# TissueImageAnalytics/cerberus

Hardware: AMD Instinct MI355X
Metric: Mpx/sec WSI tiled inference (all heads) (higher is better)
Workload: dtype f32

## Files before the change

cerberus_amd/build.py:

```python
import os
import subprocess
import sys

HERE = os.path.dirname(os.path.abspath(__file__))
CSRC = os.path.join(HERE, "csrc")
LIB = os.path.join(HERE, "libcerberus_hip.so")
LIB_DEV = os.path.join(HERE, "libcerberus_hip_dev.so")
LIB_HOST = os.path.join(HERE, "libcerberus_host.so")
HOST_SOURCES = ["host_codecs.c"]
SOURCES = ["conv_igemm.hip", "conv_wino.hip", "conv_wino4.hip", "conv_wino4b.hip", "conv_wino4p.hip", "net_kernels.hip", "postproc.hip", "slide_kernels.hip", "train_kernels.hip", "head_train.hip", "conv_wgrad.hip", "conv_wgrad_wino.hip", "pack_kernels.hip", "targets.hip", "valid_stats.hip", "jpeg_kernels.hip", "tissue_mask.hip", "cerb_api.hip", "cerb_train.hip"]
DEV_SOURCES = ["cerb_api.hip", "cerb_train.hip", "postproc.hip", "conv_wino4b.hip", "train_kernels.hip", "net_kernels.hip"]
DEV_ONLY_SOURCES = ["dev_entry.hip"]
FLAGS = ["--offload-arch=gfx950", "-O3", "-std=c++17", "-fPIC", "-Wall", "-Wno-unused-function", "-Wno-unused-result"]
EXTRA_FLAGS = {"conv_wino4.hip": ["-mllvm", "-pragma-unroll-threshold=1000000", "-mllvm", "-amdgpu-mfma-vgpr-form"],
               "conv_wino4b.hip": ["-mllvm", "-pragma-unroll-threshold=1000000"],
               "conv_wino4p.hip": ["-mllvm", "-pragma-unroll-threshold=1000000"]}


def _stale(target, deps):
    if not os.path.exists(target):
        return True
    t = os.path.getmtime(target)
    return any(os.path.getmtime(d) > t for d in deps if os.path.exists(d))


def build_host(force=False, verbose=True):
    srcs = [os.path.join(CSRC, f) for f in HOST_SOURCES]
    if force or _stale(LIB_HOST, srcs + [os.path.join(os.path.dirname(HERE), "include", "cerberus_host.h")]):
        cmd = [os.environ.get("CC", "gcc"), "-O3", "-std=c11", "-fPIC", "-shared", "-Wall", "-Wextra", "-pthread", "-o", LIB_HOST] + srcs + ["-lz"]
        if verbose:
            print(" ".join(cmd), flush=True)
        subprocess.check_call(cmd)
    return LIB_HOST


def build(force=False, verbose=True):
    build_host(force, verbose)
    hipcc = os.environ.get("HIPCC", "/opt/rocm/bin/hipcc")
    headers = [os.path.join(CSRC, f) for f in os.listdir(CSRC) if f.endswith(".h")]
    headers.append(os.path.join(os.path.dirname(HERE), "include", "cerberus_hip.h"))
    objs = []
    procs = []
    for src in SOURCES:
        sp = os.path.join(CSRC, src)
        if not os.path.exists(sp):
            continue
        obj = os.path.join(CSRC, src.replace(".hip", ".o"))
        objs.append(obj)
        if force or _stale(obj, [sp] + headers):
            cmd = [hipcc] + FLAGS + EXTRA_FLAGS.get(src, []) + ["-c", sp, "-o", obj]
            if verbose:
                print(" ".join(cmd), flush=True)
            procs.append((src, subprocess.Popen(cmd)))
    dev_objs = list(objs)
    for src in DEV_SOURCES:
        sp = os.path.join(CSRC, src)
        if not os.path.exists(sp):
            continue
        obj = os.path.join(CSRC, "dev_" + src.replace(".hip", ".o"))
        dev_objs[dev_objs.index(os.path.join(CSRC, src.replace(".hip", ".o")))] = obj
        if force or _stale(obj, [sp] + headers):
            cmd = [hipcc] + FLAGS + ["-DCERB_DEV_SWITCHES"] + EXTRA_FLAGS.get(src, []) + ["-c", sp, "-o", obj]
            if verbose:
                print(" ".join(cmd), flush=True)
            procs.append((src + " (dev)", subprocess.Popen(cmd)))
    for src in DEV_ONLY_SOURCES:
        sp = os.path.join(CSRC, src)
        obj = os.path.join(CSRC, "dev_" + src.replace(".hip", ".o"))
        dev_objs.append(obj)
        if force or _stale(obj, [sp] + headers):
            cmd = [hipcc] + FLAGS + ["-DCERB_DEV_SWITCHES"] + EXTRA_FLAGS.get(src, []) + ["-c", sp, "-o", obj]
            if verbose:
                print(" ".join(cmd), flush=True)
            procs.append((src + " (dev)", subprocess.Popen(cmd)))
    for src, p in procs:
        if p.wait() != 0:
            raise RuntimeError("hipcc failed on %s" % src)
    for lib, lobjs in ((LIB, objs), (LIB_DEV, dev_objs)):
        if force or procs or _stale(lib, lobjs):
            cmd = [hipcc, "--offload-arch=gfx950", "-shared", "-fPIC", "-o", lib] + lobjs
            if verbose:
                print(" ".join(cmd), flush=True)
            subprocess.check_call(cmd)
    return LIB


if __name__ == "__main__":
    build(force="--force" in sys.argv)
    print(LIB)
```

cerberus_amd/csrc/cerb_api.hip:

```cpp
#include "cerb_net.h"

static thread_local std::string g_err;
int cerb_set_error(const std::string& m) {
    g_err = m;
    return 1;
}
extern "C" int cerb_version(void) { return 1; }
extern "C" const char* cerb_last_error(void) { return g_err.c_str(); }
std::atomic<long long> g_devbuf_bytes{0};
extern "C" size_t cerb_device_bytes_held(void) { const long long v = g_devbuf_bytes.load(); return v > 0 ? (size_t)v : 0; }
thread_local hipStream_t g_call_stream = nullptr;

static int alloc_dev(cerb_net* net, size_t bytes, void** out) {
    if (net->reusing) {
        if (net->reuse_cursor >= net->n_finalize_allocs || net->dev_alloc_bytes[net->reuse_cursor] != bytes)
            return fail("reload: the tensors do not have the shapes the handle was finalized with");
        *out = net->dev_allocs[net->reuse_cursor++];
        return 0;
    }
    void* d = nullptr;
    HIP_OK(hipMalloc(&d, bytes));
    net->dev_allocs.push_back(d);
    net->dev_alloc_bytes.push_back(bytes);
    *out = d;
// ... 541 lines not shown
        if (!out) return 0;
    }
    const double fl = 2.0 * (double)c.groups * N * p.Ho * p.Wo * (double)c.cout * c.cin * c.ks * c.ks;
    const long long map_px = (long long)p.Ho * p.Wo;
    const bool use_w4 = net->conv_algo == 5 || net->conv_algo == 7 || (net->conv_algo == 6 && map_px >= 256);
    const bool planar = planar_out_gs > 0;
    static const long long w4b_max_px = [] {
        const char* e = cerb_dev_getenv("CERB_W4B_MAX_PX");
        return e ? atoll(e) : 4096ll;
    }();
    const bool w4b = !planar && (net->conv_algo == 7 || (net->conv_algo == 6 && map_px <= w4b_max_px)) && c.cin % 64 == 0;
    if (planar && !(use_w4 && c.wino && mode == 0 && net->fold_bn && !resid)) return fail("internal: conv " + name + " cannot take the planar path");
    if (use_w4 && c.wino && mode == 0 && (!it->second.host_w.empty() || !net->fold_bn)) {
        PackedConv& cm = it->second;
        float* train_slot = nullptr;
        if (!net->fold_bn && train_wino4_slot(net, name, cm, w4b ? 1 : 0, 0, st, &train_slot)) return 1;
        float*& slot4 = !net->fold_bn ? train_slot : (w4b ? cm.wino4b : cm.wino4);
        if (!slot4) {
            std::vector<float> w4;
            for (int g = 0; g < cm.groups; ++g) pack_wino4(cm.host_w.data() + (size_t)g * cm.cout * cm.cin * 9, cm.cout, cm.cin, &w4, w4b ? 1 : 0);
            void* d = nullptr;
            HIP_OK(hipMalloc(&d, w4.size() * 4));
            net->dev_allocs.push_back(d);
            net->dev_alloc_bytes.push_back(w4.size() * 4);
            HIP_OK(hipMemcpy(d, w4.data(), w4.size() * 4, hipMemcpyHostToDevice));
            slot4 = (float*)d;
        }
        p.wpack = slot4;
        p.w_gs = (long long)c.cout * c.cin * 36;
        double fl_done = fl;
        if (roi && roi[1] > roi[0] && roi[3] > roi[2]) {
            p.roi_y0 = roi[0]; p.roi_y1 = roi[1]; p.roi_x0 = roi[2]; p.roi_x1 = roi[3];
            const double ty = (roi[1] + 15) / 16 - roi[0] / 16, tx = (roi[3] + 15) / 16 - roi[2] / 16;
            fl_done = fl * (ty * 16.0 * tx * 16.0) / ((double)p.Ho * p.Wo);
        }
        if (planar) {
            p.out_gs = planar_out_gs;
            p.level_tag = net->planar_half ? 0 : 1;
            p.pl_byp = cerb_planar_blocks(p.Ho);
            p.pl_bxp = cerb_planar_blocks(p.Wo);
        }
        if (prof_begin(net, name, planar ? (p.level_tag ? "conv_wino4p<f4x4,16x16x2,planar>" : "conv_wino4p<f4x4,16x16x2,planar,half-res>") : w4b ? (cerb_wino4b_packed(p) ? (resid ? "conv_wino4b<f4x4,16t,res>" : "conv_wino4b<f4x4,16t>") : (resid ? "conv_wino4b<f4x4,16x16,res>" : "conv_wino4b<f4x4,16x16>")) : (resid ? "conv_wino4<f4x4,16x16x2,res>" : "conv_wino4<f4x4,16x16x2>"), fl_done, st)) return 1;
        if (net->conv_bn_part && !planar && !resid && !(roi && roi[1] > roi[0] && roi[3] > roi[2])) {
            p.bn_part = net->conv_bn_part;
            net->conv_bn_bpg = w4b ? cerb_wino4b_bn_blocks(p) : N * ((p.Ho + 15) / 16) * ((p.Wo + 15) / 16);
        }
        HIP_OK(planar ? cerb_launch_wino4p(p, st) : w4b ? cerb_launch_wino4b(p, st) : cerb_launch_wino4(p, st));
        if (prof_end(net, st)) return 1;
        return 0;
    }
    if (net->conv_algo && c.wino && mode == 0) {
        if (train_wino2_fresh(net, name, it->second, 0, st)) return 1;
        p.wpack = c.wino;
        p.w_gs = (long long)c.cout * c.cin * 16;
        double fl_done = fl;
        if (roi && roi[1] > roi[0] && roi[3] > roi[2]) {
            p.roi_y0 = roi[0]; p.roi_y1 = roi[1]; p.roi_x0 = roi[2]; p.roi_x1 = roi[3];
            const double ty = (roi[1] + 7) / 8 - roi[0] / 8, tx = (roi[3] + 15) / 16 - roi[2] / 16;
            fl_done = fl * (ty * 8.0 * tx * 16.0) / ((double)p.Ho * p.Wo);
        }
        if (prof_begin(net, name, resid ? "conv_wino<f2x2,8x16,res>" : "conv_wino<f2x2,8x16>", fl_done, st)) return 1;
        HIP_OK(cerb_launch_wino(p, st));
        if (prof_end(net, st)) return 1;
        return 0;
    }
    const std::string kn = "conv_igemm<ks" + std::to_string(c.ks) + ",s" + std::to_string(c.stride) + ",mode" + std::to_string(mode) +
                           (p.Wo < 32 ? ",16x16>" : ",8x32>");
    if (prof_begin(net, name, kn, fl, st)) return 1;
    HIP_OK(cerb_launch_conv(p, c.ks, c.stride, mode, st));
    if (prof_end(net, st)) return 1;
    return 0;
}

static int forward_impl(cerb_net* net, const cerb_forward_io* io, hipStream_t st, double* macs) {
    g_call_stream = st;
    const bool dry = (macs != nullptr) && (io->tiles == nullptr) && (io->tiles_f32 == nullptr);
    const int N = io->n, H = io->h, W = io->w;
    if (N <= 0 || H <= 0 || W <= 0 || (H % 16) || (W % 16)) return fail("cerb_net_forward: tile H,W must be positive multiples of 16");
    const int out_h = io->out_h > 0 ? io->out_h : H, out_w = io->out_w > 0 ? io->out_w : W;
    if (out_h > H || out_w > W) return fail("cerb_net_forward: crop larger than tile");
    const int hs[5] = {H, H / 2, H / 4, H / 8, H / 16}, ws[5] = {W, W / 2, W / 4, W / 8, W / 16};
    const size_t D = net->trunk_idx.size();
    const size_t guard = cerb_conv_guard_bytes(W);
    auto level_is_planar = [&](int u) {
        if (dry || u < 2 || !net->planar || !net->fold_bn || net->conv_algo != 6 || net->head_algo < 1) return false;
        const std::string n0 = "dec." + std::to_string(u) + ".0", n1 = "dec." + std::to_string(u) + ".1";
        auto c0 = net->conv.find(n0), c1 = net->conv.find(n1);
        if (c0 == net->conv.end() || c1 == net->conv.end() || !c0->second.wino) return false;
        return (long long)hs[3 - u] * ws[3 - u] > 4096 && c0->second.cin == 64 && c0->second.cout == 64 && c1->second.cout == 64;
    };
    if (!dry) {
        if (net->x0.ensure((size_t)N * H * W * 64 * 4, guard) || net->pool.ensure((size_t)N * hs[1] * ws[1] * 64 * 4, guard)) return fail_alloc();
        for (int i = 1; i < 5; ++i)
            if (net->x[i].ensure((size_t)N * hs[i] * ws[i] * kFilters[i] * 4, guard)) return fail_alloc();
        if (net->ta.ensure((size_t)N * hs[1] * ws[1] * 64 * 4, guard) || net->tb.ensure((size_t)N * hs[1] * ws[1] * 64 * 4, guard) ||
            net->cm.ensure((size_t)N * hs[4] * ws[4] * 256 * 4, guard))
            return fail_alloc();
        if (D) {
            static const bool exact_ws = cerb_dev_getenv("CERB_LEGACY_WS") == nullptr;
            size_t need_sum = 0, need_mid = 0;
            const int oc[4] = {128, 64, 64, 64};
            for (int u = 0; u < 4; ++u) {
                if (exact_ws && level_is_planar(u)) continue;
                const std::string n0 = "dec." + std::to_string(u) + ".0";
                auto c0 = net->conv.find(n0);
                const size_t px = (size_t)D * N * hs[3 - u] * ws[3 - u];
                need_sum = std::max(need_sum, px * (size_t)(c0 != net->conv.end() ? c0->second.cin : 256) * 4);
                need_mid = std::max(need_mid, px * (size_t)(c0 != net->conv.end() ? c0->second.cout : 256) * 4);
            }
            if (!exact_ws) need_sum = need_mid = D * (size_t)N * H * W * 64 * 4;
            if (net->dmid.ensure(need_mid, guard)) return fail_alloc();
            if (net->conv_algo && net->dsum.ensure(need_sum, guard)) return fail_alloc();
            for (int u = 0; u < 4; ++u) {
                if (exact_ws && level_is_planar(u)) continue;
                if (net->dout[u].ensure(D * (size_t)N * hs[3 - u] * ws[3 - u] * oc[u] * 4, guard)) return fail_alloc();
            }
        }
    }
    if (macs) *macs += (double)N * H * W * 64.0 * 147.0;
    if (!dry) {
        StemParams sp;
        sp.tiles = io->tiles; sp.tiles_f32 = io->tiles ? nullptr : io->tiles_f32; sp.wpack = net->stem_w; sp.bias = net->stem_b; sp.out = net->x0.p; sp.N = N; sp.H = H; sp.W = W; sp.relu = 1;
        sp.tiles_x = sp.tiles_y = 0;
        if (prof_begin(net, "stem", "stem_conv7x7", 2.0 * N * H * W * 64.0 * 147.0, st)) return 1;
        HIP_OK(cerb_launch_stem(sp, st));
        if (prof_end(net, st)) return 1;
        if (prof_begin(net, "maxpool", "maxpool3x3s2", 0.0, st)) return 1;
        HIP_OK(cerb_launch_maxpool(net->x0.p, net->pool.p, N, H, W, 64, st));
        if (prof_end(net, st)) return 1;
    }
    float* cur = dry ? nullptr : net->pool.p;
    int inpl = 64;
    for (int li = 0; li < 4; ++li) {
        const int planes = kFilters[li + 1];
        const int Hi = (li == 0) ? hs[1] : hs[li], Wi = (li == 0) ? ws[1] : ws[li];
        for (int b = 0; b < kLayers[li]; ++b) {
            const std::string p = "backbone.layer" + std::to_string(li + 1) + "." + std::to_string(b);
            const int stride = (b == 0 && li > 0) ? 2 : 1;
            const int hin = (b == 0) ? Hi : hs[li + 1], win = (b == 0) ? Wi : ws[li + 1];
            float* t1 = dry ? nullptr : net->ta.p;
            const bool last = (b == kLayers[li] - 1);
            float* outb = dry ? nullptr : (((kLayers[li] - 1 - b) % 2 == 0) ? net->x[li + 1].p : net->tb.p);
            (void)last;
            const float* idt = cur;
            if (run_conv(net, p + ".conv1", cur, nullptr, nullptr, t1, N, hin, win, 1, 0, 0, 0, st, macs)) return 1;
            if (stride != 1 || inpl != planes) {
                float* ds = dry ? nullptr : net->pool.p;
                if (run_conv(net, p + ".downsample", cur, nullptr, nullptr, ds, N, hin, win, 0, 0, 0, 0, st, macs)) return 1;
                idt = ds;
            }
            if (run_conv(net, p + ".conv2", t1, nullptr, idt, outb, N, hs[li + 1], ws[li + 1], 1, 0, 0, 0, st, macs)) return 1;
            cur = outb;
            inpl = planes;
        }
    }
    if (run_conv(net, "conv_map", dry ? nullptr : net->x[4].p, nullptr, nullptr, dry ? nullptr : net->cm.p, N, hs[4], ws[4], 0, 0, 0, 0, st, macs)) return 1;

    const long long tile_stride = io->tile_stride ? io->tile_stride : (long long)out_h * out_w;
    const long long row_stride = io->row_stride ? io->row_stride : out_w;
    if (net->pc_idx >= 0) {
        if (macs) *macs += (double)N * (512.0 * 256 + 256.0 * net->dec[net->pc_idx].out_ch);
        const bool want = io->out && io->out[net->pc_idx];
        const bool wantl = io->logits && io->logits[net->pc_idx];
        if (!dry && (want || wantl)) {
            PatchClassParams pp;
            memset(&pp, 0, sizeof(pp));
            pp.x4 = net->x[4].p; pp.bn1_s = net->pc_bn1s; pp.bn1_b = net->pc_bn1b; pp.w1t = net->pc_w1t; pp.b1 = net->pc_b1;
            pp.w2t = net->pc_w2t; pp.b2 = net->pc_b2;
            pp.N = N; pp.Hf = hs[4]; pp.Wf = ws[4]; pp.out_ch = net->dec[net->pc_idx].out_ch;
            pp.out_h = out_h; pp.out_w = out_w;
            pp.logits = wantl ? io->logits[net->pc_idx] : nullptr;
            pp.out = want ? (float*)io->out[net->pc_idx] : nullptr;
            pp.tile_off = io->tile_off; pp.tile_stride = tile_stride; pp.row_stride = row_stride;
            if (prof_begin(net, "patch_class", "patch_class", 2.0 * N * (512.0 * 256 + 256.0 * pp.out_ch), st)) return 1;
            HIP_OK(cerb_launch_patch_class(pp, st));
            if (prof_end(net, st)) return 1;
        }
    }
    if (D) {
        const float* skips[4] = {dry ? nullptr : net->x[3].p, dry ? nullptr : net->x[2].p, dry ? nullptr : net->x[1].p, dry ? nullptr : net->x0.p};
        const float* prev = dry ? nullptr : net->cm.p;
        long long prev_gs = 0;
        const int oc[4] = {128, 64, 64, 64};
        int roi_out[4][4], roi_mid[4][4], roi_sum[4][4];
        const bool any_logits = [&] {
            if (!io->logits) return false;
            for (size_t k = 0; k < net->dec.size(); ++k)
                if (io->logits[k]) return true;
            return false;
        }();
        const bool use_roi = !dry && net->crop_roi && (net->conv_algo == 1 || net->conv_algo >= 5) && !any_logits && (out_h < H || out_w < W);
        if (use_roi) {
            int y0 = (int)((H - out_h) * 0.5), x0 = (int)((W - out_w) * 0.5), y1 = y0 + out_h, x1 = x0 + out_w;
            for (int u = 3; u >= 0; --u) {
                const int hh = hs[3 - u], ww = ws[3 - u];
                auto widen = [&](int* r, const int* in, int d) {
                    r[0] = std::max(0, (in[0] - d) & ~3); r[1] = std::min(hh, (in[1] + d + 3) & ~3);
                    r[2] = std::max(0, (in[2] - d) & ~3); r[3] = std::min(ww, (in[3] + d + 3) & ~3);
                };
                const int win[4] = {y0, y1, x0, x1};
                widen(roi_out[u], win, 0);
                widen(roi_mid[u], roi_out[u], 1);
                widen(roi_sum[u], roi_mid[u], 1);
                y0 = std::max(0, roi_sum[u][0] / 2 - 1); y1 = std::min(hh / 2, (roi_sum[u][1] - 1) / 2 + 2);
                x0 = std::max(0, roi_sum[u][2] / 2 - 1); x1 = std::min(ww / 2, (roi_sum[u][3] - 1) / 2 + 2);
            }
        }
        bool feat_planar = false, prev_planar = false;
        for (int u = 0; u < 4; ++u) {
            const int hh = hs[3 - u], ww = ws[3 - u];
            const std::string n0 = "dec." + std::to_string(u) + ".0", n1 = "dec." + std::to_string(u) + ".1";
            const int cmid = net->conv[n0].cout;
            const int cin0 = net->conv[n0].cin;
            const bool lvl_planar = level_is_planar(u) && (u == 3 || prev_gs > 0);
            if (lvl_planar) {
                PlanarBuf &bs = u == 3 ? net->psum : net->psum2, &bm = u == 3 ? net->pmid : net->pmid2, &bo = bs;
                if (bs.ensure((int)D, N, hh, ww, 64, st) || bm.ensure((int)D, N, hh, ww, 64, st)) return fail_alloc();
                if (prof_begin(net, n0 + ".up", "upsample2_add_planar", 0.0, st)) return 1;
                HIP_OK(cerb_launch_upsample2_add_planar(skips[u], prev, bs.b.p, (int)D, N, hh, ww, cin0, prev_gs, bs.gs(), use_roi ? roi_sum[u] : nullptr, prev_planar ? 1 : 0, st));
                if (prof_end(net, st)) return 1;
                net->planar_half = (u != 3);
                if (run_conv(net, n0, bs.b.p, nullptr, nullptr, bm.b.p, N, hh, ww, 1, 0, bs.gs(), 0, st, macs, use_roi ? roi_mid[u] : nullptr, bm.gs()))
                    return 1;
                if (run_conv(net, n1, bm.b.p, nullptr, nullptr, bo.b.p, N, hh, ww, 1, 0, bm.gs(), 0, st, macs, use_roi ? roi_out[u] : nullptr, bo.gs()))
                    return 1;
                if (u == 3) feat_planar = true;
                prev = bo.b.p;
                prev_gs = bo.gs();
                prev_planar = true;
                continue;
            }
            if (prev_planar) return fail("internal: a tile-planar decoder level feeds an NHWC one");
            if (net->conv_algo && net->conv[n0].wino && !dry) {
                if (prof_begin(net, n0 + ".up", "upsample2_add", 0.0, st)) return 1;
                HIP_OK(cerb_launch_upsample2_add(skips[u], prev, net->dsum.p, (int)D, N, hh, ww, cin0, prev_gs, use_roi ? roi_sum[u] : nullptr, st));
                if (prof_end(net, st)) return 1;
                if (run_conv(net, n0, net->dsum.p, nullptr, nullptr, net->dmid.p, N, hh, ww, 1, 0, (long long)N * hh * ww * cin0, 0, st, macs,
                             use_roi ? roi_mid[u] : nullptr))
                    return 1;
            } else if (run_conv(net, n0, skips[u], prev, nullptr, dry ? nullptr : net->dmid.p, N, hh, ww, 1, 1, 0, prev_gs, st, macs)) return 1;
            if (run_conv(net, n1, dry ? nullptr : net->dmid.p, nullptr, nullptr, dry ? nullptr : net->dout[u].p, N, hh, ww, 1, 0,
                         (long long)N * hh * ww * cmid, 0, st, macs, use_roi ? roi_out[u] : nullptr))
                return 1;
            prev = dry ? nullptr : net->dout[u].p;
            prev_gs = (long long)N * hh * ww * oc[u];
        }
        HeadParams hps[8];
        int n_hp = 0;
        double head_flops = 0.0;
        for (size_t k = 0; k < net->dense_idx.size(); ++k) {
            const int di = net->dense_idx[k];
            const size_t tk = (size_t)net->trunk_of[k];
            const DecoderCfg& d = net->dec[di];
            if (macs) *macs += (double)N * H * W * (64.0 * 96 + 96.0 * d.out_ch);
            const bool want = io->out && io->out[di];
            const bool wantl = io->logits && io->logits[di];
            if (dry || !(want || wantl)) continue;
            HeadParams hp;
            memset(&hp, 0, sizeof(hp));
            hp.feat = feat_planar ? net->psum.b.p + tk * net->psum.gs() : net->dout[3].p + tk * (size_t)N * H * W * 64;
            hp.feat_planar = feat_planar ? 1 : 0;
            hp.pl_byp = cerb_planar_blocks(H);
            hp.pl_bxp = cerb_planar_blocks(W);
            hp.w1p = net->head_w1[k]; hp.b1 = net->head_b1[k]; hp.w2p = net->head_w2[k]; hp.b2 = net->head_b2[k]; hp.w2q = net->head_w2q[k];
            hp.N = N; hp.H = H; hp.W = W; hp.out_ch = d.out_ch; hp.kind = d.kind;
            hp.crop_y0 = (int)((H - out_h) * 0.5); hp.crop_x0 = (int)((W - out_w) * 0.5);
            hp.out_h = want ? out_h : 0; hp.out_w = want ? out_w : 0;
            hp.roi = use_roi ? 1 : 0;
            hp.logits = wantl ? io->logits[di] : nullptr;
            hp.absmax_bits = io->logit_absmax ? io->logit_absmax + di : nullptr;
            if (want) {
                if (d.kind == 0) hp.out_inst = (float*)io->out[di];
                else if (io->type_is_u8) hp.out_type_u8 = (unsigned char*)io->out[di];
                else hp.out_type_i64 = (long long*)io->out[di];
            }
            hp.tile_off = io->tile_off; hp.tile_stride = tile_stride; hp.row_stride = row_stride;
            const double head_px = hp.roi ? (double)out_h * (((hp.crop_x0 + out_w + 15) / 16 - hp.crop_x0 / 16) * 16.0) : (double)H * W;
            const double fl = 2.0 * N * head_px * (64.0 * 96 + 96.0 * d.out_ch);
            if (net->head_algo == 0) {
                if (prof_begin(net, "head." + d.name, "head", fl, st)) return 1;
                HIP_OK(cerb_launch_head(hp, st));
                if (prof_end(net, st)) return 1;
            } else {
                if (n_hp == 8) {
                    if (prof_begin(net, "heads", "head_group", head_flops, st)) return 1;
                    HIP_OK(cerb_launch_head_group(hps, n_hp, st, net->head_algo == 1 ? 1 : 0));
                    if (prof_end(net, st)) return 1;
                    n_hp = 0;
                    head_flops = 0.0;
                }
                hps[n_hp++] = hp;
                head_flops += fl;
            }
        }
        if (n_hp > 0) {
            if (prof_begin(net, "heads", "head_group", head_flops, st)) return 1;
            HIP_OK(cerb_launch_head_group(hps, n_hp, st, net->head_algo == 1 ? 1 : 0));
            if (prof_end(net, st)) return 1;
        }
    }
    if (!dry && io->feats) {
        const float* src[6] = {net->x0.p, net->x[1].p, net->x[2].p, net->x[3].p, net->cm.p, net->x[4].p};
        const size_t nb[6] = {(size_t)N * H * W * 64, (size_t)N * hs[1] * ws[1] * 64, (size_t)N * hs[2] * ws[2] * 128,
                              (size_t)N * hs[3] * ws[3] * 256, (size_t)N * hs[4] * ws[4] * 256, (size_t)N * hs[4] * ws[4] * 512};
        for (int i = 0; i < 6; ++i)
            if (io->feats[i]) HIP_OK(hipMemcpyAsync(io->feats[i], src[i], nb[i] * 4, hipMemcpyDeviceToDevice, st));
    }
    return 0;
}

extern "C" int cerb_net_begin_reload(cerb_net* net) {
    if (!net) return fail("cerb_net_begin_reload: null handle");
    HIP_OK(hipDeviceSynchronize());
    while (net->dev_allocs.size() > net->n_finalize_allocs) {
        (void)hipFree(net->dev_allocs.back());
        net->dev_allocs.pop_back();
        net->dev_alloc_bytes.pop_back();
    }
    net->reusing = true;
    net->reuse_cursor = 0;
// ... 195 lines not shown
```

cerberus_amd/csrc/net_kernels.hip:

```cpp
#include "cerb_common.h"

struct StemParams {
    const unsigned char* tiles;
    const float* tiles_f32;
    const float* wpack;
    const float* bias;
    float* out;
    int N, H, W, tiles_x, tiles_y;
    int relu;
};

template <bool F32IN>
__global__ __launch_bounds__(256, 2) void stem_conv7x7_kernel(StemParams p) {
    constexpr int TH = 8, TW = 32, IH = TH + 6, IW = TW + 6, ROW = 120;
    __shared__ __attribute__((aligned(16))) float wl[7 * 12 * 2 * 64];
    __shared__ __attribute__((aligned(16))) float xl[IH * ROW];
    const int tid = threadIdx.x, lane = tid & 63, wave = tid >> 6, j = lane & 31, h = lane >> 5;
    for (int i = tid; i < 7 * 12 * 2 * 64; i += 256) wl[i] = p.wpack[i];
    const int ntile = p.N * p.tiles_y * p.tiles_x;
    for (int tile = blockIdx.x; tile < ntile; tile += gridDim.x) {
        int t_ = tile;
        const int tx = t_ % p.tiles_x;
        t_ /= p.tiles_x;
        const int ty = t_ % p.tiles_y;
        const int n = t_ / p.tiles_y;
        const int oy0 = ty * TH, ox0 = tx * TW;
        __syncthreads();
        const unsigned char* img = F32IN ? nullptr : p.tiles + (long long)n * p.H * p.W * 3;
        const float* imgf = F32IN ? p.tiles_f32 + (long long)n * p.H * p.W * 3 : nullptr;
        for (int i = tid; i < IH * ROW; i += 256) {
            const int iy = i / ROW, c = i % ROW;
            const int gy = oy0 - 3 + iy, gx = ox0 - 3 + c / 3;
            float v = 0.f;
            if (c < IW * 3 && gy >= 0 && gy < p.H && gx >= 0 && gx < p.W) {
                const long long at = ((long long)gy * p.W + gx) * 3 + c % 3;
                v = (F32IN ? imgf[at] : (float)img[at]) / 255.0f;
            }
            xl[i] = v;
        }
        __syncthreads();
        f32x16 acc[2][2];
#pragma unroll
        for (int s = 0; s < 2; ++s)
#pragma unroll
            for (int q = 0; q < 2; ++q)
#pragma unroll
                for (int r = 0; r < 16; ++r) acc[s][q][r] = 0.f;
        const int b0 = (wave * 2 + 0) * ROW + j * 3 + h;
        const int b1 = (wave * 2 + 1) * ROW + j * 3 + h;
#pragma unroll
        for (int ky = 0; ky < 7; ++ky) {
#pragma unroll
            for (int t = 0; t < 12; ++t) {
                const float a0 = wl[((ky * 12 + t) * 2 + 0) * 64 + lane];
                const float a1 = wl[((ky * 12 + t) * 2 + 1) * 64 + lane];
                const float x0 = xl[b0 + ky * ROW + 2 * t];
                const float x1 = xl[b1 + ky * ROW + 2 * t];
                acc[0][0] = __builtin_amdgcn_mfma_f32_32x32x2f32(a0, x0, acc[0][0], 0, 0, 0);
                acc[1][0] = __builtin_amdgcn_mfma_f32_32x32x2f32(a1, x0, acc[1][0], 0, 0, 0);
                acc[0][1] = __builtin_amdgcn_mfma_f32_32x32x2f32(a0, x1, acc[0][1], 0, 0, 0);
                acc[1][1] = __builtin_amdgcn_mfma_f32_32x32x2f32(a1, x1, acc[1][1], 0, 0, 0);
            }
        }
#pragma unroll
        for (int q = 0; q < 2; ++q) {
            const int oy = oy0 + wave * 2 + q, ox = ox0 + j;
            if (oy >= p.H || ox >= p.W) continue;
            float* o = p.out + (((long long)n * p.H + oy) * p.W + ox) * 64;
#pragma unroll
            for (int s = 0; s < 2; ++s)
#pragma unroll
                for (int rq = 0; rq < 4; ++rq) {
                    const int co = s * 32 + rq * 8 + h * 4;
                    f32x4 v = {acc[s][q][rq * 4 + 0], acc[s][q][rq * 4 + 1], acc[s][q][rq * 4 + 2], acc[s][q][rq * 4 + 3]};
                    v = v + *reinterpret_cast<const f32x4*>(p.bias + co);
                    const float floor_ = p.relu ? 0.f : -3.402823466e38f;
                    v[0] = fmaxf(v[0], floor_);
                    v[1] = fmaxf(v[1], floor_);
                    v[2] = fmaxf(v[2], floor_);
                    v[3] = fmaxf(v[3], floor_);
                    *reinterpret_cast<f32x4*>(o + co) = v;
                }
        }
    }
}

hipError_t cerb_launch_stem(StemParams p, hipStream_t st) {
    p.tiles_x = (p.W + 31) / 32;
    p.tiles_y = (p.H + 7) / 8;
    const long long ntile = (long long)p.N * p.tiles_x * p.tiles_y;
    const unsigned grid = (unsigned)(ntile < 256 * 6 ? ntile : 256 * 6);
    if (p.tiles) hipLaunchKernelGGL(stem_conv7x7_kernel<false>, dim3(grid), dim3(256), 0, st, p);
    else hipLaunchKernelGGL(stem_conv7x7_kernel<true>, dim3(grid), dim3(256), 0, st, p);
    return hipGetLastError();
}

__global__ void maxpool3x3s2_kernel(const float* __restrict__ in, float* __restrict__ out, int N, int H, int W, int C, int Ho, int Wo) {
    const long long total = (long long)N * Ho * Wo * (C / 4);
    const long long per_xcd = gridDim.x / 8, vb = (long long)(blockIdx.x & 7) * per_xcd + (blockIdx.x >> 3);
    for (long long i = vb * (long long)blockDim.x + threadIdx.x; i < total; i += (long long)gridDim.x * blockDim.x) {
        const int c4 = (int)(i % (C / 4));
        long long r = i / (C / 4);
        const int ox = (int)(r % Wo);
        r /= Wo;
        const int oy = (int)(r % Ho);
        const int n = (int)(r / Ho);
        f32x4 m = {-INFINITY, -INFINITY, -INFINITY, -INFINITY};
#pragma unroll
        for (int ky = 0; ky < 3; ++ky) {
            const int y = oy * 2 - 1 + ky;
            if (y < 0 || y >= H) continue;
#pragma unroll
            for (int kx = 0; kx < 3; ++kx) {
                const int x = ox * 2 - 1 + kx;
                if (x < 0 || x >= W) continue;
                const f32x4 v = *reinterpret_cast<const f32x4*>(in + (((long long)n * H + y) * W + x) * C + c4 * 4);
                m[0] = fmaxf(m[0], v[0]);
                m[1] = fmaxf(m[1], v[1]);
                m[2] = fmaxf(m[2], v[2]);
                m[3] = fmaxf(m[3], v[3]);
            }
        }
        *reinterpret_cast<f32x4*>(out + i * 4) = m;
    }
}

__global__ void maxpool3x3s2_idx_kernel(const float* __restrict__ in, float* __restrict__ out, unsigned* __restrict__ idx, int N, int H, int W, int C, int Ho, int Wo) {
    const long long total = (long long)N * Ho * Wo * (C / 4);
    const long long per_xcd = gridDim.x / 8, vb = (long long)(blockIdx.x & 7) * per_xcd + (blockIdx.x >> 3);
    for (long long i = vb * (long long)blockDim.x + threadIdx.x; i < total; i += (long long)gridDim.x * blockDim.x) {
        const int c4 = (int)(i % (C / 4));
        long long r = i / (C / 4);
        const int ox = (int)(r % Wo);
        r /= Wo;
        const int oy = (int)(r % Ho);
        const int n = (int)(r / Ho);
        f32x4 m = {-INFINITY, -INFINITY, -INFINITY, -INFINITY};
        unsigned w0 = 0, w1 = 0, w2 = 0, w3 = 0;
        bool first = true;
#pragma unroll
        for (int ky = 0; ky < 3; ++ky) {
            const int y = oy * 2 - 1 + ky;
            if (y < 0 || y >= H) continue;
#pragma unroll
            for (int kx = 0; kx < 3; ++kx) {
                const int x = ox * 2 - 1 + kx;
                if (x < 0 || x >= W) continue;
                const f32x4 v = *reinterpret_cast<const f32x4*>(in + (((long long)n * H + y) * W + x) * C + c4 * 4);
                const unsigned k = (unsigned)(ky * 3 + kx);
                if (first || v[0] > m[0]) w0 = k;
                if (first || v[1] > m[1]) w1 = k;
                if (first || v[2] > m[2]) w2 = k;
                if (first || v[3] > m[3]) w3 = k;
                first = false;
                m[0] = fmaxf(m[0], v[0]);
                m[1] = fmaxf(m[1], v[1]);
                m[2] = fmaxf(m[2], v[2]);
                m[3] = fmaxf(m[3], v[3]);
            }
        }
        *reinterpret_cast<f32x4*>(out + i * 4) = m;
        idx[i] = w0 | (w1 << 8) | (w2 << 16) | (w3 << 24);
    }
}

hipError_t cerb_launch_maxpool_idx(const float* in, float* out, unsigned* idx, int N, int H, int W, int C, hipStream_t st) {
    const int Ho = (H + 2 - 3) / 2 + 1, Wo = (W + 2 - 3) / 2 + 1;
    const long long total = (long long)N * Ho * Wo * (C / 4);
    long long blocks = ((total + 255) / 256 + 7) / 8 * 8;
    if (blocks > 256 * 64) blocks = 256 * 64;
    hipLaunchKernelGGL(maxpool3x3s2_idx_kernel, dim3((unsigned)blocks), dim3(256), 0, st, in, out, idx, N, H, W, C, Ho, Wo);
    return hipGetLastError();
}

// ... 647 lines not shown
    }
    if (p.absmax_bits) head_absmax_commit(p.absmax_bits, amax);
}

template <bool W2_44>
__global__ __launch_bounds__(256, HEAD_G_OCC) void head_group_kernel(HeadGroupParams gp) {
    __shared__ __attribute__((aligned(16))) float s_w1[6 * 4 * 64 * 4];
    __shared__ __attribute__((aligned(16))) float s_w2[(W2_44 ? 2 : 1) * 6 * 64 * 4];
    __shared__ __attribute__((aligned(16))) float s_b1[96];
    __shared__ __attribute__((aligned(16))) float s_b2[32];
    const HeadParams& p = gp.h[blockIdx.y];
    const bool generic = !W2_44 || gp.generic || p.logits != nullptr;
    const int shape = generic ? 0 : p.kind * 8 + p.out_ch;
    const bool spec = shape == 2 || shape == 3 || shape == 8 + 3 || shape == 8 + 7;
    {
        const int tid = threadIdx.x;
        const f32x4h* w1g = reinterpret_cast<const f32x4h*>(p.w1p);
        const f32x4h* w2g = reinterpret_cast<const f32x4h*>(W2_44 ? p.w2q : p.w2p);
        const int w2n = (W2_44 && !(spec && p.out_ch <= 4) ? 2 : 1) * 6 * 64;
        for (int i = tid; i < 6 * 4 * 64; i += 256) reinterpret_cast<f32x4h*>(s_w1)[i] = w1g[i];
        for (int i = tid; i < w2n; i += 256) reinterpret_cast<f32x4h*>(s_w2)[i] = w2g[i];
        if (tid < 96) s_b1[tid] = p.b1[tid];
        if (tid < 32) s_b2[tid] = p.b2[tid];
    }
    __syncthreads();
    if constexpr (W2_44) {
        if (shape == 2) return head_group_body<true, 2, 0>(p, s_w1, s_w2, s_b1, s_b2);
        if (shape == 3) return head_group_body<true, 3, 0>(p, s_w1, s_w2, s_b1, s_b2);
        if (shape == 8 + 3) return head_group_body<true, 3, 1>(p, s_w1, s_w2, s_b1, s_b2);
        if (shape == 8 + 7) return head_group_body<true, 7, 1>(p, s_w1, s_w2, s_b1, s_b2);
    }
    head_group_body<W2_44, 0, 0>(p, s_w1, s_w2, s_b1, s_b2);
}

hipError_t cerb_launch_head_group(const HeadParams* heads, int n_heads, hipStream_t st, int w2_44) {
    if (n_heads < 1 || n_heads > 8) return hipErrorInvalidValue;

    HeadGroupParams gp = {};
    gp.n_heads = n_heads;
#ifdef CERB_DEV_SWITCHES
    {
        const char* e = cerb_dev_getenv("CERB_HEAD_GENERIC");
        gp.generic = e && e[0] != '0';
    }
#endif
    unsigned max_blocks = 0;
    for (int i = 0; i < n_heads; ++i) {
        HeadParams p = heads[i];
        if (p.W % 16) return hipErrorInvalidValue;
        p.rows = p.H; p.row0 = 0; p.xa0 = 0; p.nxb = p.W / 16;
        if (p.roi && !p.logits && p.out_h > 0 && p.out_w > 0) {
            p.rows = p.out_h; p.row0 = p.crop_y0;
            p.xa0 = p.crop_x0 & ~15;
            p.nxb = (p.crop_x0 + p.out_w - p.xa0 + 15) / 16;
        }
        const long long nblk = (long long)p.N * p.rows * p.nxb;
        if (nblk >= (1ll << 31)) return hipErrorInvalidValue;
        const long long ntask = (nblk + 1) / 2;
        const long long blocks = (ntask + 4 * HEAD_G_TPW - 1) / (4 * HEAD_G_TPW);
        if (blocks > max_blocks) max_blocks = (unsigned)blocks;
        gp.h[i] = p;
    }
    if (w2_44) hipLaunchKernelGGL(head_group_kernel<true>, dim3(max_blocks, (unsigned)n_heads), dim3(256), 0, st, gp);
    else hipLaunchKernelGGL(head_group_kernel<false>, dim3(max_blocks, (unsigned)n_heads), dim3(256), 0, st, gp);
    return hipGetLastError();
}

struct PatchClassParams {
    const float* x4;
    const float* bn1_s;
    const float* bn1_b;
    const float* w1t;
    const float* b1;
    const float* w2t;
    const float* b2;
    int N, Hf, Wf, out_ch;
    int out_h, out_w;
    float* logits;
    float* out;
    const long long* tile_off;
    long long tile_stride, row_stride;
};

__global__ __launch_bounds__(256) void patch_class_kernel(PatchClassParams p) {
    __shared__ float v[512];
    __shared__ float hid[256];
    __shared__ float lg[16];
    __shared__ int cls_s;
    const int n = blockIdx.x, tid = threadIdx.x;
    int y0 = 0, x0 = 0, ch = p.Hf, cw = p.Wf;
    if (p.Hf != 9 && p.Wf != 9) {
        auto py_slice = [](int len, int& start, int& count) {
            const int h0 = (int)((len - 9) * 0.5);
            const int a0 = h0 < 0 ? max(len + h0, 0) : min(h0, len);
            const int a1 = min(h0 + 9, len);
            start = a0;
            count = max(a1 - a0, 0);
        };
        py_slice(p.Hf, y0, ch);
        py_slice(p.Wf, x0, cw);
    }
    const float* x = p.x4 + (long long)n * p.Hf * p.Wf * 512;
    for (int c = tid; c < 512; c += 256) {
        float s = 0.f;
        for (int yy = 0; yy < ch; ++yy)
            for (int xx = 0; xx < cw; ++xx) s += x[((long long)(y0 + yy) * p.Wf + (x0 + xx)) * 512 + c];
        s = s / (float)(ch * cw);
        s = s * p.bn1_s[c] + p.bn1_b[c];
        v[c] = fmaxf(s, 0.f);
    }
    __syncthreads();
    {
        float s = 0.f;
        for (int c = 0; c < 512; ++c) s = fmaf(p.w1t[c * 256 + tid], v[c], s);
        hid[tid] = fmaxf(s + p.b1[tid], 0.f);
    }
    __syncthreads();
    if (tid < 16) {
        float s = 0.f;
        if (tid < p.out_ch) {
            for (int c = 0; c < 256; ++c) s = fmaf(p.w2t[c * 16 + tid], hid[c], s);
            s += p.b2[tid];
            if (p.logits) p.logits[n * p.out_ch + tid] = s;
        }
        lg[tid] = s;
    }
    __syncthreads();
    if (tid == 0) {
        float mx = lg[0];
        for (int e = 1; e < p.out_ch; ++e) mx = fmaxf(mx, lg[e]);
        float sum = 0.f, ex[16];
        for (int e = 0; e < p.out_ch; ++e) {
            ex[e] = expf(lg[e] - mx);
            sum += ex[e];
        }
        int best = 0;
        float bv = ex[0] / sum;
        for (int e = 1; e < p.out_ch; ++e) {
            const float pe = ex[e] / sum;
            if (pe > bv) {
                bv = pe;
                best = e;
            }
        }
        cls_s = best;
    }
    __syncthreads();
    if (p.out) {
        const float cf = (float)cls_s;
        const long long base = p.tile_off ? p.tile_off[n] : (long long)n * p.tile_stride;
        for (int i = tid; i < p.out_h * p.out_w; i += 256) {
            const int yy = i / p.out_w, xx = i % p.out_w;
            p.out[base + (long long)yy * p.row_stride + xx] = cf;
        }
    }
}

hipError_t cerb_launch_patch_class(const PatchClassParams& p, hipStream_t st) {
    hipLaunchKernelGGL(patch_class_kernel, dim3(p.N), dim3(256), 0, st, p);
    return hipGetLastError();
}
```

Measured before the change: 149.1.

## Pipeline stem conv loads, share decoder level-0 sum, split patch-class fill

The stem 7x7 conv now prefetches the next tile's input into registers while MFMA runs on the current one, and uses a shared-memory byte-to-float table. Decoder level 0 builds one upsample-add sum shared across all decoder branches instead of one per branch when the previous stage is not grouped, which cuts memory traffic and workspace. The patch-class kernel batches its loads for more memory-level parallelism and hands the output fill to a separate wide kernel. This adds an extra launch and more register pressure in the stem, and old paths stay behind dev switches.

```diff
diff --git a/cerberus_amd/build.py b/cerberus_amd/build.py
--- a/cerberus_amd/build.py
+++ b/cerberus_amd/build.py
@@ -10,7 +10,7 @@
 HOST_SOURCES = ["host_codecs.c"]
 SOURCES = ["conv_igemm.hip", "conv_wino.hip", "conv_wino4.hip", "conv_wino4b.hip", "conv_wino4p.hip", "net_kernels.hip", "postproc.hip", "slide_kernels.hip", "train_kernels.hip", "head_train.hip", "conv_wgrad.hip", "conv_wgrad_wino.hip", "pack_kernels.hip", "targets.hip", "valid_stats.hip", "jpeg_kernels.hip", "tissue_mask.hip", "cerb_api.hip", "cerb_train.hip"]
 DEV_SOURCES = ["cerb_api.hip", "cerb_train.hip", "postproc.hip", "conv_wino4b.hip", "train_kernels.hip", "net_kernels.hip"]
-DEV_ONLY_SOURCES = ["dev_entry.hip"]
+DEV_ONLY_SOURCES = ["dev_entry.hip", "dev_entry_fwd.hip"]
 FLAGS = ["--offload-arch=gfx950", "-O3", "-std=c++17", "-fPIC", "-Wall", "-Wno-unused-function", "-Wno-unused-result"]
 EXTRA_FLAGS = {"conv_wino4.hip": ["-mllvm", "-pragma-unroll-threshold=1000000", "-mllvm", "-amdgpu-mfma-vgpr-form"],
                "conv_wino4b.hip": ["-mllvm", "-pragma-unroll-threshold=1000000"],
diff --git a/cerberus_amd/csrc/cerb_api.hip b/cerberus_amd/csrc/cerb_api.hip
--- a/cerberus_amd/csrc/cerb_api.hip
+++ b/cerberus_amd/csrc/cerb_api.hip
@@ -647,6 +647,13 @@
     const int hs[5] = {H, H / 2, H / 4, H / 8, H / 16}, ws[5] = {W, W / 2, W / 4, W / 8, W / 16};
     const size_t D = net->trunk_idx.size();
     const size_t guard = cerb_conv_guard_bytes(W);
+    bool entry0_shared = true;
+#ifdef CERB_DEV_SWITCHES
+    {
+        const char* e = cerb_dev_getenv("CERB_ENTRY0_PRIVATE");
+        if (e && e[0] != '0') entry0_shared = false;
+    }
+#endif
     auto level_is_planar = [&](int u) {
         if (dry || u < 2 || !net->planar || !net->fold_bn || net->conv_algo != 6 || net->head_algo < 1) return false;
         const std::string n0 = "dec." + std::to_string(u) + ".0", n1 = "dec." + std::to_string(u) + ".1";
@@ -670,7 +677,7 @@
                 const std::string n0 = "dec." + std::to_string(u) + ".0";
                 auto c0 = net->conv.find(n0);
                 const size_t px = (size_t)D * N * hs[3 - u] * ws[3 - u];
-                need_sum = std::max(need_sum, px * (size_t)(c0 != net->conv.end() ? c0->second.cin : 256) * 4);
+                need_sum = std::max(need_sum, (u == 0 && entry0_shared ? px / D : px) * (size_t)(c0 != net->conv.end() ? c0->second.cin : 256) * 4);
                 need_mid = std::max(need_mid, px * (size_t)(c0 != net->conv.end() ? c0->second.cout : 256) * 4);
             }
             if (!exact_ws) need_sum = need_mid = D * (size_t)N * H * W * 64 * 4;
@@ -798,9 +805,10 @@
             if (prev_planar) return fail("internal: a tile-planar decoder level feeds an NHWC one");
             if (net->conv_algo && net->conv[n0].wino && !dry) {
                 if (prof_begin(net, n0 + ".up", "upsample2_add", 0.0, st)) return 1;
-                HIP_OK(cerb_launch_upsample2_add(skips[u], prev, net->dsum.p, (int)D, N, hh, ww, cin0, prev_gs, use_roi ? roi_sum[u] : nullptr, st));
+                const bool one_sum = entry0_shared && prev_gs == 0;
+                HIP_OK(cerb_launch_upsample2_add(skips[u], prev, net->dsum.p, one_sum ? 1 : (int)D, N, hh, ww, cin0, prev_gs, use_roi ? roi_sum[u] : nullptr, st));
                 if (prof_end(net, st)) return 1;
-                if (run_conv(net, n0, net->dsum.p, nullptr, nullptr, net->dmid.p, N, hh, ww, 1, 0, (long long)N * hh * ww * cin0, 0, st, macs,
+                if (run_conv(net, n0, net->dsum.p, nullptr, nullptr, net->dmid.p, N, hh, ww, 1, 0, one_sum ? 0 : (long long)N * hh * ww * cin0, 0, st, macs,
                              use_roi ? roi_mid[u] : nullptr))
                     return 1;
             } else if (run_conv(net, n0, skips[u], prev, nullptr, dry ? nullptr : net->dmid.p, N, hh, ww, 1, 1, 0, prev_gs, st, macs)) return 1;
diff --git a/cerberus_amd/csrc/dev_entry_fwd.hip b/cerberus_amd/csrc/dev_entry_fwd.hip
--- /dev/null
+++ b/cerberus_amd/csrc/dev_entry_fwd.hip
@@ -0,0 +1,25 @@
+#include "cerb_net.h"
+
+extern "C" {
+
+int cerb_fwdtest_stem(const unsigned char* tiles, const float* tiles_f32, const float* wpack, const float* bias, float* out, int N, int H, int W, int relu, void* st) {
+    if (!(tiles || tiles_f32) || !wpack || !bias || !out || N <= 0 || H <= 0 || W <= 0) return (int)hipErrorInvalidValue;
+    StemParams sp;
+    sp.tiles = tiles; sp.tiles_f32 = tiles ? nullptr : tiles_f32; sp.wpack = wpack; sp.bias = bias; sp.out = out;
+    sp.N = N; sp.H = H; sp.W = W; sp.tiles_x = sp.tiles_y = 0; sp.relu = relu;
+    return (int)cerb_launch_stem(sp, (hipStream_t)st);
+}
+
+int cerb_fwdtest_patch_class(const float* x4, const float* bn1_s, const float* bn1_b, const float* w1t, const float* b1, const float* w2t, const float* b2, int N, int Hf,
+                             int Wf, int out_ch, int out_h, int out_w, float* logits, float* out, const long long* tile_off, long long tile_stride,
+                             long long row_stride, void* st) {
+    if (!x4 || !bn1_s || !bn1_b || !w1t || !b1 || !w2t || !b2 || N <= 0 || Hf <= 0 || Wf <= 0 || out_ch < 1 || out_ch > 16 || out_h <= 0 || out_w <= 0)
+        return (int)hipErrorInvalidValue;
+    PatchClassParams pp;
+    pp.x4 = x4; pp.bn1_s = bn1_s; pp.bn1_b = bn1_b; pp.w1t = w1t; pp.b1 = b1; pp.w2t = w2t; pp.b2 = b2;
+    pp.N = N; pp.Hf = Hf; pp.Wf = Wf; pp.out_ch = out_ch; pp.out_h = out_h; pp.out_w = out_w;
+    pp.logits = logits; pp.out = out; pp.tile_off = tile_off; pp.tile_stride = tile_stride; pp.row_stride = row_stride;
+    return (int)cerb_launch_patch_class(pp, (hipStream_t)st);
+}
+
+}
diff --git a/cerberus_amd/csrc/net_kernels.hip b/cerberus_amd/csrc/net_kernels.hip
--- a/cerberus_amd/csrc/net_kernels.hip
+++ b/cerberus_amd/csrc/net_kernels.hip
@@ -10,12 +10,166 @@
     int relu;
 };
 
+constexpr int STEM_TH = 8, STEM_TW = 32, STEM_IH = STEM_TH + 6, STEM_IW = STEM_TW + 6, STEM_ROW = 120;
+
+__device__ __forceinline__ void stem_tile_mma(const StemParams& p, const float* wl, const float* xl, int n, int oy0, int ox0, int lane, int wave) {
+    constexpr int ROW = STEM_ROW;
+    const int j = lane & 31, h = lane >> 5;
+    f32x16 acc[2][2];
+#pragma unroll
+    for (int s = 0; s < 2; ++s)
+#pragma unroll
+        for (int q = 0; q < 2; ++q)
+#pragma unroll
+            for (int r = 0; r < 16; ++r) acc[s][q][r] = 0.f;
+    const int b0 = (wave * 2 + 0) * ROW + j * 3 + h;
+    const int b1 = (wave * 2 + 1) * ROW + j * 3 + h;
+#pragma unroll
+    for (int ky = 0; ky < 7; ++ky) {
+#pragma unroll
+        for (int t = 0; t < 12; ++t) {
+            const float a0 = wl[((ky * 12 + t) * 2 + 0) * 64 + lane];
+            const float a1 = wl[((ky * 12 + t) * 2 + 1) * 64 + lane];
+            const float x0 = xl[b0 + ky * ROW + 2 * t];
+            const float x1 = xl[b1 + ky * ROW + 2 * t];
+            acc[0][0] = __builtin_amdgcn_mfma_f32_32x32x2f32(a0, x0, acc[0][0], 0, 0, 0);
+            acc[1][0] = __builtin_amdgcn_mfma_f32_32x32x2f32(a1, x0, acc[1][0], 0, 0, 0);
+            acc[0][1] = __builtin_amdgcn_mfma_f32_32x32x2f32(a0, x1, acc[0][1], 0, 0, 0);
+            acc[1][1] = __builtin_amdgcn_mfma_f32_32x32x2f32(a1, x1, acc[1][1], 0, 0, 0);
+        }
+    }
+#pragma unroll
+    for (int q = 0; q < 2; ++q) {
+        const int oy = oy0 + wave * 2 + q, ox = ox0 + j;
+        if (oy >= p.H || ox >= p.W) continue;
+        float* o = p.out + (((long long)n * p.H + oy) * p.W + ox) * 64;
+#pragma unroll
+        for (int s = 0; s < 2; ++s)
+#pragma unroll
+            for (int rq = 0; rq < 4; ++rq) {
+                const int co = s * 32 + rq * 8 + h * 4;
+                f32x4 v = {acc[s][q][rq * 4 + 0], acc[s][q][rq * 4 + 1], acc[s][q][rq * 4 + 2], acc[s][q][rq * 4 + 3]};
+                v = v + *reinterpret_cast<const f32x4*>(p.bias + co);
+                const float floor_ = p.relu ? 0.f : -3.402823466e38f;
+                v[0] = fmaxf(v[0], floor_);
+                v[1] = fmaxf(v[1], floor_);
+                v[2] = fmaxf(v[2], floor_);
+                v[3] = fmaxf(v[3], floor_);
+                *reinterpret_cast<f32x4*>(o + co) = v;
+            }
+    }
+}
+
 template <bool F32IN>
 __global__ __launch_bounds__(256, 2) void stem_conv7x7_kernel(StemParams p) {
-    constexpr int TH = 8, TW = 32, IH = TH + 6, IW = TW + 6, ROW = 120;
+    constexpr int IH = STEM_IH, ROW = STEM_ROW, ROWE = STEM_IW * 3, NWORD = 30;
+    constexpr int NSLOT = F32IN ? (IH * ROWE + 255) / 256 : (IH * NWORD + 255) / 256, PER_ROW = F32IN ? ROWE : NWORD;
     __shared__ __attribute__((aligned(16))) float wl[7 * 12 * 2 * 64];
     __shared__ __attribute__((aligned(16))) float xl[IH * ROW];
-    const int tid = threadIdx.x, lane = tid & 63, wave = tid >> 6, j = lane & 31, h = lane >> 5;
+    __shared__ float tab[256];
+    const int tid = threadIdx.x, lane = tid & 63, wave = tid >> 6;
+    for (int i = tid; i < 7 * 12 * 2 * 64; i += 256) wl[i] = p.wpack[i];
+    for (int i = tid; i < IH * ROW; i += 256) xl[i] = 0.f;
+    tab[tid] = (float)tid / 255.0f;
+    int s_row[NSLOT], s_pos[NSLOT];
+#pragma unroll
+    for (int k = 0; k < NSLOT; ++k) {
+        const int idx = tid + 256 * k;
+        s_row[k] = idx < IH * PER_ROW ? idx / PER_ROW : -1;
+        s_pos[k] = F32IN ? idx % PER_ROW : (idx % PER_ROW) * 4;
+    }
+    unsigned r_word[NSLOT];
+    [[maybe_unused]] int r_meta[NSLOT];
+    const int ntile = p.N * p.tiles_y * p.tiles_x, W3 = p.W * 3;
+    const long long total = (long long)p.N * p.H * W3;
+
+    auto fetch = [&](int tile) {
+        int t_ = tile;
+        const int tx = t_ % p.tiles_x;
+        t_ /= p.tiles_x;
+        const int ty = t_ % p.tiles_y;
+        const int n = t_ / p.tiles_y;
+        const int r0 = (tx * STEM_TW - 3) * 3;
+#pragma unroll
+        for (int k = 0; k < NSLOT; ++k) {
+            if (s_row[k] < 0) continue;
+            const int gy = ty * STEM_TH - 3 + s_row[k];
+            const bool row_ok = gy >= 0 && gy < p.H;
+            const long long rowoff = ((long long)n * p.H + gy) * W3;
+            if constexpr (F32IN) {
+                const int q = r0 + s_pos[k];
+                float v = 0.f;
+                if (row_ok && q >= 0 && q < W3) v = p.tiles_f32[rowoff + q];
+                r_word[k] = __float_as_uint(v);
+            } else {
+                const int mis = (int)(((unsigned long long)p.tiles + (unsigned long long)(rowoff + r0)) & 3);
+                const int c0 = s_pos[k] - mis, q0 = r0 + c0;
+                unsigned m = 0, w = 0;
+#pragma unroll
+                for (int b = 0; b < 4; ++b)
+                    if (row_ok && q0 + b >= 0 && q0 + b < W3 && c0 + b >= 0 && c0 + b < ROWE) m |= 1u << b;
+                if (m) {
+                    const long long off = rowoff + q0;
+                    if (off >= 0 && off + 4 <= total) {
+                        w = *reinterpret_cast<const unsigned*>(p.tiles + off);
+                    } else {
+#pragma unroll
+                        for (int b = 0; b < 4; ++b)
+                            if (m >> b & 1) w |= (unsigned)p.tiles[off + b] << (8 * b);
+                    }
+                }
+                r_word[k] = w;
+                r_meta[k] = (c0 + 4) | (int)(m << 8);
+            }
+        }
+    };
+    auto commit = [&](float* buf) {
+#pragma unroll
+        for (int k = 0; k < NSLOT; ++k) {
+            if (s_row[k] < 0) continue;
+            float* row = buf + s_row[k] * ROW;
+            if constexpr (F32IN) {
+                row[s_pos[k]] = __uint_as_float(r_word[k]) / 255.0f;
+            } else {
+                const int c0 = (r_meta[k] & 255) - 4;
+                const unsigned m = (unsigned)r_meta[k] >> 8;
+#pragma unroll
+                for (int b = 0; b < 4; ++b) {
+                    const int c = c0 + b;
+                    if (c >= 0 && c < ROWE) row[c] = (m >> b & 1) ? tab[(r_word[k] >> (8 * b)) & 255] : 0.f;
+                }
+            }
+        }
+    };
+
+    int tile = blockIdx.x;
+    fetch(tile);
+    __syncthreads();
+    commit(xl);
+    for (; tile < ntile; tile += gridDim.x) {
+        const int next = tile + gridDim.x;
+        __syncthreads();
+        if (next < ntile) fetch(next);
+        int t_ = tile;
+        const int tx = t_ % p.tiles_x;
+        t_ /= p.tiles_x;
+        const int ty = t_ % p.tiles_y;
+        const int n = t_ / p.tiles_y;
+        stem_tile_mma(p, wl, xl, n, ty * STEM_TH, tx * STEM_TW, lane, wave);
+        if (next < ntile) {
+            __syncthreads();
+            commit(xl);
+        }
+    }
+}
+
+#ifdef CERB_DEV_SWITCHES
+template <bool F32IN>
+__global__ __launch_bounds__(256, 2) void stem_conv7x7_old_kernel(StemParams p) {
+    constexpr int TH = STEM_TH, TW = STEM_TW, IH = STEM_IH, IW = STEM_IW, ROW = STEM_ROW;
+    __shared__ __attribute__((aligned(16))) float wl[7 * 12 * 2 * 64];
+    __shared__ __attribute__((aligned(16))) float xl[IH * ROW];
+    const int tid = threadIdx.x, lane = tid & 63, wave = tid >> 6;
     for (int i = tid; i < 7 * 12 * 2 * 64; i += 256) wl[i] = p.wpack[i];
     const int ntile = p.N * p.tiles_y * p.tiles_x;
     for (int tile = blockIdx.x; tile < ntile; tile += gridDim.x) {
@@ -39,57 +193,26 @@
             xl[i] = v;
         }
         __syncthreads();
-        f32x16 acc[2][2];
-#pragma unroll
-        for (int s = 0; s < 2; ++s)
-#pragma unroll
-            for (int q = 0; q < 2; ++q)
-#pragma unroll
-                for (int r = 0; r < 16; ++r) acc[s][q][r] = 0.f;
-        const int b0 = (wave * 2 + 0) * ROW + j * 3 + h;
-        const int b1 = (wave * 2 + 1) * ROW + j * 3 + h;
-#pragma unroll
-        for (int ky = 0; ky < 7; ++ky) {
-#pragma unroll
-            for (int t = 0; t < 12; ++t) {
-                const float a0 = wl[((ky * 12 + t) * 2 + 0) * 64 + lane];
-                const float a1 = wl[((ky * 12 + t) * 2 + 1) * 64 + lane];
-                const float x0 = xl[b0 + ky * ROW + 2 * t];
-                const float x1 = xl[b1 + ky * ROW + 2 * t];
-                acc[0][0] = __builtin_amdgcn_mfma_f32_32x32x2f32(a0, x0, acc[0][0], 0, 0, 0);
-                acc[1][0] = __builtin_amdgcn_mfma_f32_32x32x2f32(a1, x0, acc[1][0], 0, 0, 0);
-                acc[0][1] = __builtin_amdgcn_mfma_f32_32x32x2f32(a0, x1, acc[0][1], 0, 0, 0);
-                acc[1][1] = __builtin_amdgcn_mfma_f32_32x32x2f32(a1, x1, acc[1][1], 0, 0, 0);
-            }
-        }
-#pragma unroll
-        for (int q = 0; q < 2; ++q) {
-            const int oy = oy0 + wave * 2 + q, ox = ox0 + j;
-            if (oy >= p.H || ox >= p.W) continue;
-            float* o = p.out + (((long long)n * p.H + oy) * p.W + ox) * 64;
-#pragma unroll
-            for (int s = 0; s < 2; ++s)
-#pragma unroll
-                for (int rq = 0; rq < 4; ++rq) {
-                    const int co = s * 32 + rq * 8 + h * 4;
-                    f32x4 v = {acc[s][q][rq * 4 + 0], acc[s][q][rq * 4 + 1], acc[s][q][rq * 4 + 2], acc[s][q][rq * 4 + 3]};
-                    v = v + *reinterpret_cast<const f32x4*>(p.bias + co);
-                    const float floor_ = p.relu ? 0.f : -3.402823466e38f;
-                    v[0] = fmaxf(v[0], floor_);
-                    v[1] = fmaxf(v[1], floor_);
-                    v[2] = fmaxf(v[2], floor_);
-                    v[3] = fmaxf(v[3], floor_);
-                    *reinterpret_cast<f32x4*>(o + co) = v;
-                }
-        }
-    }
-}
+        stem_tile_mma(p, wl, xl, n, oy0, ox0, lane, wave);
+    }
+}
+#endif
 
 hipError_t cerb_launch_stem(StemParams p, hipStream_t st) {
     p.tiles_x = (p.W + 31) / 32;
     p.tiles_y = (p.H + 7) / 8;
     const long long ntile = (long long)p.N * p.tiles_x * p.tiles_y;
     const unsigned grid = (unsigned)(ntile < 256 * 6 ? ntile : 256 * 6);
+#ifdef CERB_DEV_SWITCHES
+    {
+        const char* e = cerb_dev_getenv("CERB_STEM_OLD");
+        if (e && e[0] != '0') {
+            if (p.tiles) hipLaunchKernelGGL(stem_conv7x7_old_kernel<false>, dim3(grid), dim3(256), 0, st, p);
+            else hipLaunchKernelGGL(stem_conv7x7_old_kernel<true>, dim3(grid), dim3(256), 0, st, p);
+            return hipGetLastError();
+        }
+    }
+#endif
     if (p.tiles) hipLaunchKernelGGL(stem_conv7x7_kernel<false>, dim3(grid), dim3(256), 0, st, p);
     else hipLaunchKernelGGL(stem_conv7x7_kernel<true>, dim3(grid), dim3(256), 0, st, p);
     return hipGetLastError();
@@ -903,13 +1026,8 @@
     long long tile_stride, row_stride;
 };
 
-__global__ __launch_bounds__(256) void patch_class_kernel(PatchClassParams p) {
-    __shared__ float v[512];
-    __shared__ float hid[256];
-    __shared__ float lg[16];
-    __shared__ int cls_s;
-    const int n = blockIdx.x, tid = threadIdx.x;
-    int y0 = 0, x0 = 0, ch = p.Hf, cw = p.Wf;
+__device__ __forceinline__ void patch_class_window(const PatchClassParams& p, int& y0, int& x0, int& ch, int& cw) {
+    y0 = 0, x0 = 0, ch = p.Hf, cw = p.Wf;
     if (p.Hf != 9 && p.Wf != 9) {
         auto py_slice = [](int len, int& start, int& count) {
             const int h0 = (int)((len - 9) * 0.5);
@@ -921,6 +1039,119 @@
         py_slice(p.Hf, y0, ch);
         py_slice(p.Wf, x0, cw);
     }
+}
+
+__device__ __forceinline__ void patch_class_argmax(const PatchClassParams& p, const float* lg, int* cls_s) {
+    float mx = lg[0];
+    for (int e = 1; e < p.out_ch; ++e) mx = fmaxf(mx, lg[e]);
+    float sum = 0.f, ex[16];
+    for (int e = 0; e < p.out_ch; ++e) {
+        ex[e] = expf(lg[e] - mx);
+        sum += ex[e];
+    }
+    int best = 0;
+    float bv = ex[0] / sum;
+    for (int e = 1; e < p.out_ch; ++e) {
+        const float pe = ex[e] / sum;
+        if (pe > bv) {
+            bv = pe;
+            best = e;
+        }
+    }
+    *cls_s = best;
+}
+
+__global__ __launch_bounds__(256) void patch_class_kernel(PatchClassParams p) {
+    __shared__ float v[512];
+    __shared__ float hid[256];
+    __shared__ float lg[16];
+    __shared__ int cls_s;
+    const int n = blockIdx.x, tid = threadIdx.x;
+    int y0, x0, ch, cw;
+    patch_class_window(p, y0, x0, ch, cw);
+    const float* x = p.x4 + (long long)n * p.Hf * p.Wf * 512;
+    {
+        float s[2] = {0.f, 0.f};
+        const int cnt = ch * cw;
+        int ly = 0, lx = 0;
+        for (int base = 0; base < cnt; base += 27) {
+            float r[27][2];
+#pragma unroll
+            for (int j = 0; j < 27; ++j)
+                if (base + j < cnt) {
+                    const float* px = x + ((long long)(y0 + ly) * p.Wf + (x0 + lx)) * 512 + tid;
+                    r[j][0] = px[0];
+                    r[j][1] = px[256];
+                    if (++lx == cw) lx = 0, ++ly;
+                }
+#pragma unroll
+            for (int j = 0; j < 27; ++j)
+                if (base + j < cnt) {
+                    s[0] += r[j][0];
+                    s[1] += r[j][1];
+                }
+        }
+#pragma unroll
+        for (int k = 0; k < 2; ++k) {
+            const int c = tid + 256 * k;
+            float t = s[k] / (float)(ch * cw);
+            t = t * p.bn1_s[c] + p.bn1_b[c];
+            v[c] = fmaxf(t, 0.f);
+        }
+    }
+    __syncthreads();
+    {
+        float s = 0.f;
+        for (int c0 = 0; c0 < 512; c0 += 64) {
+            float w[64];
+#pragma unroll
+            for (int i = 0; i < 64; ++i) w[i] = p.w1t[(c0 + i) * 256 + tid];
+#pragma unroll
+            for (int i = 0; i < 64; ++i) s = fmaf(w[i], v[c0 + i], s);
+        }
+        hid[tid] = fmaxf(s + p.b1[tid], 0.f);
+    }
+    __syncthreads();
+    if (tid < 16) {
+        float s = 0.f;
+        if (tid < p.out_ch) {
+            for (int c0 = 0; c0 < 256; c0 += 16) {
+                float w[16];
+#pragma unroll
+                for (int i = 0; i < 16; ++i) w[i] = p.w2t[(c0 + i) * 16 + tid];
+#pragma unroll
+                for (int i = 0; i < 16; ++i) s = fmaf(w[i], hid[c0 + i], s);
+            }
+            s += p.b2[tid];
+            if (p.logits) p.logits[n * p.out_ch + tid] = s;
+        }
+        lg[tid] = s;
+    }
+    __syncthreads();
+    if (tid == 0) {
+        patch_class_argmax(p, lg, &cls_s);
+        if (p.out) p.out[p.tile_off ? p.tile_off[n] : (long long)n * p.tile_stride] = (float)cls_s;
+    }
+}
+
+__global__ __launch_bounds__(256) void patch_class_fill_kernel(PatchClassParams p, int per) {
+    const int n = blockIdx.x / per, tid = threadIdx.x;
+    const long long base = p.tile_off ? p.tile_off[n] : (long long)n * p.tile_stride;
+    const float cf = p.out[base];
+    for (int yy = blockIdx.x % per; yy < p.out_h; yy += per)
+        for (int xx = tid; xx < p.out_w; xx += 256)
+            if (yy | xx) p.out[base + (long long)yy * p.row_stride + xx] = cf;
+}
+
+#ifdef CERB_DEV_SWITCHES
+__global__ __launch_bounds__(256) void patch_class_old_kernel(PatchClassParams p) {
+    __shared__ float v[512];
+    __shared__ float hid[256];
+    __shared__ float lg[16];
+    __shared__ int cls_s;
+    const int n = blockIdx.x, tid = threadIdx.x;
+    int y0, x0, ch, cw;
+    patch_class_window(p, y0, x0, ch, cw);
     const float* x = p.x4 + (long long)n * p.Hf * p.Wf * 512;
     for (int c = tid; c < 512; c += 256) {
         float s = 0.f;
@@ -947,25 +1178,7 @@
         lg[tid] = s;
     }
     __syncthreads();
-    if (tid == 0) {
-        float mx = lg[0];
-        for (int e = 1; e < p.out_ch; ++e) mx = fmaxf(mx, lg[e]);
-        float sum = 0.f, ex[16];
-        for (int e = 0; e < p.out_ch; ++e) {
-            ex[e] = expf(lg[e] - mx);
-            sum += ex[e];
-        }
-        int best = 0;
-        float bv = ex[0] / sum;
-        for (int e = 1; e < p.out_ch; ++e) {
-            const float pe = ex[e] / sum;
-            if (pe > bv) {
-                bv = pe;
-                best = e;
-            }
-        }
-        cls_s = best;
-    }
+    if (tid == 0) patch_class_argmax(p, lg, &cls_s);
     __syncthreads();
     if (p.out) {
         const float cf = (float)cls_s;
@@ -976,8 +1189,22 @@
         }
     }
 }
+#endif
 
 hipError_t cerb_launch_patch_class(const PatchClassParams& p, hipStream_t st) {
+#ifdef CERB_DEV_SWITCHES
+    {
+        const char* e = cerb_dev_getenv("CERB_PATCH_CLASS_OLD");
+        if (e && e[0] != '0') {
+            hipLaunchKernelGGL(patch_class_old_kernel, dim3(p.N), dim3(256), 0, st, p);
+            return hipGetLastError();
+        }
+    }
+#endif
     hipLaunchKernelGGL(patch_class_kernel, dim3(p.N), dim3(256), 0, st, p);
+    if (p.out && p.out_h > 0 && p.out_w > 0) {
+        const int per = p.out_h < 16 ? p.out_h : 16;
+        hipLaunchKernelGGL(patch_class_fill_kernel, dim3((unsigned)p.N * (unsigned)per), dim3(256), 0, st, p, per);
+    }
     return hipGetLastError();
 }
```

Result: no change. 149.0 (-0.1%).
